# ryanelandt/PressureFieldContact.jl

Hardware: NVIDIA B200
Metric: contact_wrench_evals_per_sec (higher is better)
Workload: dtype f64

## Files before the change

pressurefieldcontact.jl_b200/csrc/pfc_clip.cuh:

```cuda
#pragma once
#include "pfc_math.cuh"
#include "pfc_types.cuh"

namespace pfc {

template <class T> struct Zeta { T c[4]; };

template <class T> PFC_D Zeta<T> clip_node(const Zeta<T>& z_non, const Zeta<T>& z_pos, int i) {
    const T w1 = z_non.c[i], w2 = z_pos.c[i];
    const T inv = 1.0 / (w1 - w2);
    const T c1 = w1 * inv, c2 = w2 * inv;
    Zeta<T> r;
#pragma unroll
    for (int k = 0; k < 4; ++k) r.c[k] = c1 * z_pos.c[k] - c2 * z_non.c[k];
    return r;
}

template <class T> __device__ __noinline__ int clip_tet(Zeta<T>* z, int n, int& flags) {
    for (int i = 0; i < 4; ++i) {
        bool all_non_pos = true, all_non_neg = true;
        unsigned non_pos = 0;
        for (int k = 0; k < n; ++k) {
            const double s = val(z[k].c[i]);
            const bool np = (s <= 0.0);
            non_pos |= (np ? 1u : 0u) << k;
            all_non_pos = all_non_pos && np;
            all_non_neg = all_non_neg && (0.0 <= s);
        }
        if (all_non_pos) return 0;
        if (all_non_neg) continue;
        int k0 = -1;
        for (int k = 0; k < n; ++k) {
            const int k1 = (k + 1 == n) ? 0 : k + 1;
            if (((non_pos >> k) & 1u) && !((non_pos >> k1) & 1u)) { k0 = k; break; }
        }
        if (k0 < 0) { flags |= kFlagNonFinite; return 0; }
        Zeta<T> w[8];
        for (int j = 0; j < n; ++j) { int k = k0 + j; if (k >= n) k -= n; w[j] = z[k]; }
        int m = n;
        while (m > 3 && val(w[m - 2].c[i]) <= 0.0) --m;
        const Zeta<T> z_start = clip_node(w[0], w[1], i);
        const double last = val(w[m - 1].c[i]);
        const bool last_inside = (m <= 5) ? (0.0 < last) : (0.0 <= last);
        z[0] = z_start;
        if (last_inside) {
            for (int k = 1; k < m; ++k) z[k] = w[k];
            z[m] = clip_node(w[0], w[m - 1], i);
            n = m + 1;
        } else {
            for (int k = 1; k < m - 1; ++k) z[k] = w[k];
            z[m - 1] = clip_node(w[m - 1], w[m - 2], i);
            n = m;
        }
        if (m == 7) return n;
    }
    return n;
}

PFC_D void clip_node_inplace(const double* zn, const double* zp, double w1, double w2, double* r) {
    const double inv = 1.0 / (w1 - w2);
    const double c1 = w1 * inv, c2 = w2 * inv;
#pragma unroll
    for (int k = 0; k < 4; ++k) r[k] = c1 * zp[k] - c2 * zn[k];
}
PFC_D int clip_tet_inplace(double* z, int n, int& flags) {
#pragma unroll 1
    for (int i = 0; i < 4; ++i) {
        unsigned np = 0, nn = 0, ps = 0;
        for (int k = 0; k < n; ++k) {
            const double s = z[4 * k + i];
            np |= (s <= 0.0 ? 1u : 0u) << k;
            nn |= (0.0 <= s ? 1u : 0u) << k;
            ps |= (0.0 < s ? 1u : 0u) << k;
        }
        const unsigned full = (1u << n) - 1u;
        if (np == full) return 0;
        if (nn == full) continue;
        const unsigned trans = np & ~(((np >> 1) | (np << (n - 1))) & full);
        if (!trans) { flags |= kFlagNonFinite; return 0; }
        const int k0 = __ffs(trans) - 1;
        const unsigned rnp = ((np >> k0) | (np << (n - k0))) & full;
        const unsigned rnn = ((nn >> k0) | (nn << (n - k0))) & full;
        const unsigned rps = ((ps >> k0) | (ps << (n - k0))) & full;
        int m = n;
        while (m > 3 && ((rnp >> (m - 2)) & 1u)) --m;
        const bool last_inside = (((m <= 5) ? rps : rnn) >> (m - 1)) & 1u;
        const int keep_end = last_inside ? m - 1 : m - 2;
        double w0[4], w1[4], wa[4], wb[4], zs[4], ze[4];
        {
            const int i1 = (k0 + 1 < n) ? k0 + 1 : k0 + 1 - n;
            const int ja = last_inside ? 0 : m - 1, jb = last_inside ? m - 1 : m - 2;
            const int ia = (k0 + ja < n) ? k0 + ja : k0 + ja - n, ib = (k0 + jb < n) ? k0 + jb : k0 + jb - n;
#pragma unroll
            for (int c = 0; c < 4; ++c) { w0[c] = z[4 * k0 + c]; w1[c] = z[4 * i1 + c]; wa[c] = z[4 * ia + c]; wb[c] = z[4 * ib + c]; }
            clip_node_inplace(w0, w1, z[4 * k0 + i], z[4 * i1 + i], zs);
            clip_node_inplace(wa, wb, z[4 * ia + i], z[4 * ib + i], ze);
        }
        if (k0 != 0) {
#pragma unroll 1
            for (int c = 0; c < 4; ++c) {
                double t[7];
#pragma unroll
                for (int j = 1; j <= 7; ++j)
                    if (j <= keep_end) { const int idx = (k0 + j < n) ? k0 + j : k0 + j - n; t[j - 1] = z[4 * idx + c]; }
#pragma unroll
                for (int j = 1; j <= 7; ++j)
                    if (j <= keep_end) z[4 * j + c] = t[j - 1];
            }
        }
#pragma unroll
        for (int c = 0; c < 4; ++c) { z[c] = zs[c]; z[4 * (keep_end + 1) + c] = ze[c]; }
        n = keep_end + 2;
        if (m == 7) return n;
    }
    return n;
}

template <class T> PFC_D void zero_small(Zeta<T>* z, int n) {
    for (int k = 0; k < n; ++k)
#pragma unroll
        for (int i = 0; i < 4; ++i) {
            const bool keep = 1.0e-14 < fabs(val(z[k].c[i]));
            z[k].c[i] = z[k].c[i] * (keep ? 1.0 : 0.0);
        }
}

template <class T> PFC_D Vec3<T> weight_poly(const Vec3<T>& p1, const Vec3<T>& p2, const T& w1, const T& w2) {
    const T inv = 1.0 / (w1 - w2);
    const T c1 = w1 * inv, c2 = w2 * inv;
    return mk<T>(c1 * p2.x - c2 * p1.x, c1 * p2.y - c2 * p1.y, c1 * p2.z - c2 * p1.z);
}

template <class T> __device__ __noinline__ int plane_tet(const T* plane, const Vec3<T>* v, Vec3<T>* out) {
    T proj[4];
    int n_neg = 0, n_pos = 0;
    unsigned pos = 0, neg = 0;
#pragma unroll
    for (int k = 0; k < 4; ++k) {
        proj[k] = plane[0] * v[k].x + plane[1] * v[k].y + plane[2] * v[k].z + plane[3];
        const double p = val(proj[k]);
        if (p < 0.0) { ++n_neg; neg |= 1u << k; }
        if (0.0 < p) { ++n_pos; pos |= 1u << k; }
    }
    if (n_pos == 0 || n_neg == 0) return 0;
    const signed char TRI[4][3][2] = {{{1, 0}, {3, 0}, {2, 0}}, {{0, 1}, {2, 1}, {3, 1}}, {{0, 2}, {3, 2}, {1, 2}}, {{0, 3}, {1, 3}, {2, 3}}};
    const signed char QUAD[3][4][2] = {{{1, 2}, {1, 3}, {0, 3}, {0, 2}}, {{0, 1}, {0, 3}, {2, 3}, {2, 1}}, {{0, 2}, {0, 1}, {3, 1}, {3, 2}}};
    int cnt, sel;
    bool forward;
    if (n_pos == 1) { sel = __ffs(pos) - 1; cnt = 3; forward = true; }
    else if (n_neg == 1) { sel = __ffs(neg) - 1; cnt = 3; forward = false; }
    else {
        const unsigned p0 = pos & 1u;
        if (((pos >> 1) & 1u) == p0) sel = 0;
        else if (((pos >> 2) & 1u) == p0) sel = 1;
        else if (((pos >> 3) & 1u) == p0) sel = 2;
        else return 0;
        cnt = 4;
        forward = (0.0 < val(proj[0]));
    }
    for (int k = 0; k < cnt; ++k) {
        const int i1 = (cnt == 3) ? TRI[sel][k][0] : QUAD[sel][k][0];
        const int i2 = (cnt == 3) ? TRI[sel][k][1] : QUAD[sel][k][1];
        const Vec3<T> p = weight_poly(v[i1], v[i2], proj[i1], proj[i2]);
        out[forward ? k : cnt - 1 - k] = p;
    }
    return cnt;
}

}
```

pressurefieldcontact.jl_b200/csrc/pfc_large.cu:

```cuda
#include <algorithm>
#include <cstddef>
#include <cstdio>
#include <cstdlib>
#include <vector>

#include <cuda_pipeline_primitives.h>

#include "pfc_exact.h"
#include "pfc_large.h"
#include "pfc_patch.cuh"
#include "pfc_sat.cuh"

namespace pfc {

namespace {

#define LCU(call)                         \
    do {                                  \
        cudaError_t e_ = (call);          \
        if (e_ != cudaSuccess) return e_; \
    } while (0)

constexpr int kStackCap = 1024;
constexpr int kDfsWarps = 4;
// ... 419 lines not shown
        unsigned incl = s;
#pragma unroll
        for (int o = 1; o < 32; o <<= 1) { const unsigned v = __shfl_up_sync(0xffffffffu, incl, o); if (lane >= o) incl += v; }
        unsigned run = incl - s;
#pragma unroll
        for (int j = 0; j < 8; ++j) { base[wib][8 * lane + j] = run + hist[(size_t)(8 * lane + j) * cap_tiles + tile]; run += t[j]; }
    }
    __syncwarp();
    const unsigned beg = tile * kTile, end = min(beg + kTile, n);
    constexpr int B = 8;
    for (unsigned c0 = beg; c0 < end; c0 += 32 * B) {
        unsigned long long kk[B]; unsigned vv[B];
#pragma unroll
        for (int j = 0; j < B; ++j) { const unsigned i = c0 + 32 * j + lane; const bool ok = i < end; kk[j] = ok ? keys_in[i] : 0ull; vv[j] = ok ? vals_in[i] : 0u; }
#pragma unroll
        for (int j = 0; j < B; ++j) {
            const unsigned i = c0 + 32 * j + lane;
            const bool valid = i < end;
            const unsigned d = valid ? (unsigned)((kk[j] >> shift) & 255u) : 256u + lane;
            const unsigned peers = __match_any_sync(0xffffffffu, d);
            const unsigned rank = __popc(peers & ((1u << lane) - 1u));
            unsigned pos = 0;
            if (valid) pos = base[wib][d] + rank;
            __syncwarp();
            if (valid && rank == (unsigned)__popc(peers) - 1) base[wib][d] = pos + 1;
            __syncwarp();
            if (valid) { keys_out[pos] = kk[j]; vals_out[pos] = vv[j]; }
        }
    }
}

__global__ void __launch_bounds__(1024) small_sort_kernel(const unsigned long long* keys_in, const unsigned* vals_in, Counters* cnt, unsigned cap_pairs,
                                                          unsigned long long* keys_out, unsigned* vals_out, int radix_queued) {
    extern __shared__ __align__(16) unsigned char sort_smem[];
    const unsigned n = listed_pairs(cnt, cap_pairs);
    if (n > kSmallSort && !radix_queued && threadIdx.x == 0) atomicOr(&cnt->overflow, 8u);
    if (n == 0 || n > kSmallSort) return;
    unsigned m = 1;
    while (m < n) m <<= 1;
    unsigned long long* k = reinterpret_cast<unsigned long long*>(sort_smem);
    unsigned* v = reinterpret_cast<unsigned*>(k + m);
    for (unsigned i = threadIdx.x; i < m; i += blockDim.x) { k[i] = i < n ? keys_in[i] : ~0ull; v[i] = i < n ? vals_in[i] : 0u; }
    __syncthreads();
    for (unsigned size = 2; size <= m; size <<= 1)
        for (unsigned stride = size >> 1; stride > 0; stride >>= 1) {
            for (unsigned t = threadIdx.x; t < m / 2; t += blockDim.x) {
                const unsigned lo = 2 * t - (t & (stride - 1)), hi = lo + stride;
                const bool up = (lo & size) == 0;
                const unsigned long long a = k[lo], b = k[hi];
                if ((a > b) == up) { k[lo] = b; k[hi] = a; const unsigned tv = v[lo]; v[lo] = v[hi]; v[hi] = tv; }
            }
            __syncthreads();
        }
    for (unsigned i = threadIdx.x; i < n; i += blockDim.x) { keys_out[i] = k[i]; vals_out[i] = v[i]; }
}

__global__ void gather_sorted_kernel(const int3* __restrict__ pairs, const unsigned* __restrict__ vals, const Counters* cnt, unsigned cap_pairs, int3* sorted,
                                     unsigned* seg_start, unsigned* seg_end) {
    const unsigned n = listed_pairs(cnt, cap_pairs);
    for (unsigned i = blockIdx.x * blockDim.x + threadIdx.x; i < n; i += gridDim.x * blockDim.x) {
        const int3 p = pairs[vals[i]];
        sorted[i] = p;
        const int prev = i > 0 ? pairs[vals[i - 1]].x : -1;
        if (p.x != prev) { seg_start[p.x] = i; if (prev >= 0) seg_end[prev] = i; }
        if (i == n - 1) seg_end[p.x] = n;
    }
}
__global__ void __launch_bounds__(1024) units_scan_kernel(const unsigned* __restrict__ seg_start, const unsigned* __restrict__ seg_end, unsigned n_prob, unsigned* unit_start,
                                                          Counters* cnt, unsigned shard_rank, unsigned shard_world) {
    __shared__ unsigned warp_sums[32];
    __shared__ unsigned carry;
    if (threadIdx.x == 0) carry = 0;
    __syncthreads();
    const int lane = threadIdx.x & 31, w = threadIdx.x >> 5;
    for (unsigned base = 0; base < n_prob; base += 1024) {
        const unsigned i = base + threadIdx.x;
        const unsigned v = i < n_prob ? (seg_end[i] - seg_start[i] + kChunk - 1) / kChunk : 0;
        unsigned incl = v;
#pragma unroll
        for (int o = 1; o < 32; o <<= 1) { const unsigned t = __shfl_up_sync(0xffffffffu, incl, o); if (lane >= o) incl += t; }
        if (lane == 31) warp_sums[w] = incl;
        __syncthreads();
        if (w == 0) {
            unsigned s = warp_sums[lane];
#pragma unroll
            for (int o = 1; o < 32; o <<= 1) { const unsigned t = __shfl_up_sync(0xffffffffu, s, o); if (lane >= o) s += t; }
            warp_sums[lane] = s;
        }
        __syncthreads();
        const unsigned before = carry + (w > 0 ? warp_sums[w - 1] : 0) + incl - v;
        if (i < n_prob) unit_start[i] = before;
        __syncthreads();
        if (threadIdx.x == 1023) carry = before + v;
        __syncthreads();
    }
    if (threadIdx.x == 0) { unit_start[n_prob] = carry; cnt->n_units = carry; }
    (void)shard_rank; (void)shard_world;
}

constexpr int kLPolyStride = 35;
static_assert(sizeof(PolyRec<double>) == kLPolyStride * sizeof(double), "PolyRec<double> is 35 doubles");
struct NarrowLargeSmem {
    double poly[kChunk * kLPolyStride];
    double item_res[kChunk * 7];
    PatchCtx<double> cx;
    double fpv[8];
    double tot[8];
    unsigned short items[kChunk * 8];
    int2 slot_pair[kChunk];
    unsigned char slot_n[kChunk];
    int warp_tot[kChunk / 32];
    int s_prob;
    int pflags;
};

__global__ void __launch_bounds__(kChunk, 2) narrow_large_kernel(SceneDev sc, LargeScene ls, EvalIO io, const int3* __restrict__ sorted, const unsigned* __restrict__ seg_start,
                                                                 const unsigned* __restrict__ seg_end, const unsigned* __restrict__ unit_start, unsigned n_prob,
                                                                 const Counters* cnt, double* chunk_out, int* chunk_points, int* prob_flags) {
    extern __shared__ __align__(16) unsigned char smem_raw[];
    NarrowLargeSmem& sm = *reinterpret_cast<NarrowLargeSmem*>(smem_raw);
    const unsigned n_units = cnt->n_units;
    const int tid = threadIdx.x, lane = tid & 31, wib = tid >> 5;
    constexpr int NW = kChunk / 32;
    for (unsigned u = blockIdx.x; u < n_units; u += gridDim.x) {
        if (tid == 0) {
            unsigned lo = 0, hi = n_prob;
            while (hi - lo > 1) { const unsigned mid = (lo + hi) >> 1; if (unit_start[mid] <= u) lo = mid; else hi = mid; }
            sm.s_prob = (int)lo;
            sm.pflags = 0;
        }
        __syncthreads();
        const int p = sm.s_prob;
        long long env; int k;
        prob_to_ei(sc, ls, p, env, k);
        const InsDev& ins = sc.ins[k];
        if (ins.model != PFC_MODEL_REGULARIZED) { __syncthreads(); continue; }
        const long long ei = env * sc.n_ins + k;
        if (wib == 0) {
            const double* X = io.X + 16 * ei;
            const double* twist = io.twist + 6 * ei;
            PatchCtx<double>& cx = sm.cx;
            if (lane < 8) sm.fpv[lane] = ins.p[lane];
            if (lane < 9) { const int i = lane / 3, j = lane % 3; cx.x21.r[lane] = X[4 * j + i]; }
            else if (lane < 12) cx.x21.t[lane - 9] = X[12 + lane - 9];
            else if (lane < 21) { const int e = lane - 12, i = e / 3, j = e % 3; cx.x12.r[e] = X[4 * i + j]; }
            else if (lane < 24) { const int i = lane - 21; cx.x12.t[i] = -(X[4 * i] * X[12] + X[4 * i + 1] * X[13] + X[4 * i + 2] * X[14]); }
            else if (lane < 27) (&cx.w_ang.x)[lane - 24] = twist[lane - 24];
            else if (lane < 30) (&cx.w_lin.x)[lane - 27] = twist[lane - 24];
            else if (lane == 30) { cx.chi = ins.chi; cx.Ebar1 = ins.Ebar1; cx.Ebar2 = ins.Ebar2; cx.n_quad = ins.n_quad; }
            if (lane < 8) sm.tot[lane] = 0.0;
        }
        __syncthreads();
        const unsigned i = seg_start[p] + (u - unit_start[p]) * kChunk + tid;
        double zr[16];
        int n0 = 0;
        int3 pr = make_int3(0, 0, 0);
        if (i < seg_end[p]) {
            pr = sorted[i];
            n0 = start_polygon_zeta(sc, ins, pr.y, pr.z, sm.cx, zr);
        }
        const unsigned alive = __ballot_sync(0xffffffffu, n0 > 0);
        if (lane == 0) sm.warp_tot[wib] = __popc(alive);
        __syncthreads();
        int before = 0, n_slot = 0;
#pragma unroll
        for (int w = 0; w < NW; ++w) { const int t = sm.warp_tot[w]; if (w < wib) before += t; n_slot += t; }
        if (n0 > 0) {
            const int slot = before + __popc(alive & ((1u << lane) - 1u));
            double* z = sm.poly + slot * kLPolyStride;
#pragma unroll
            for (int j = 0; j < 16; ++j)
                if (j < 4 * n0) z[j] = zr[j];
            sm.slot_pair[slot] = make_int2(pr.y, pr.z); sm.slot_n[slot] = (unsigned char)n0;
        }
        __syncthreads();
        int nv = 0;
        if (tid < n_slot) {
            const int2 e = sm.slot_pair[tid];
            PolyRec<double>& out = *reinterpret_cast<PolyRec<double>*>(sm.poly + tid * kLPolyStride);
            int flags = 0;
            const int n = clip_tet_inplace(reinterpret_cast<double*>(&out), (int)sm.slot_n[tid], flags);
            if (n >= 3) {
                finish_polygon_slot(n, sc.tets[ins.prim_base2 + e.y], pair_normal(sc, ins, e.x, e.y, sm.cx), out);
                nv = n;
            }
            if (flags) atomicOr(&sm.pflags, flags);
        }
        int incl = nv;
#pragma unroll
        for (int o = 1; o < 32; o <<= 1) { const int v = __shfl_up_sync(0xffffffffu, incl, o); if (lane >= o) incl += v; }
        __syncthreads();
        if (lane == 31) sm.warp_tot[wib] = incl;
        __syncthreads();
        int ibefore = 0, total = 0;
#pragma unroll
        for (int w = 0; w < NW; ++w) { const int t = sm.warp_tot[w]; if (w < wib) ibefore += t; total += t; }
        const int at = ibefore + incl - nv;
        for (int q = 0; q < nv; ++q) sm.items[at + q] = (unsigned short)((tid << 3) | q);
        __syncthreads();
        for (int i0 = 0; i0 < total; i0 += kChunk) {
            const int i1 = min(total, i0 + kChunk);
            const int it = i0 + tid;
            if (it < i1) {
                const int code = sm.items[it];
                const int slot = code >> 3, q = code & 7;
                const PolyRec<double>& prc = *reinterpret_cast<const PolyRec<double>*>(sm.poly + slot * kLPolyStride);
                Accum<double, 6> tmp;
                tmp.fp = sm.fpv; tmp.w_ang = sm.cx.w_ang; tmp.w_lin = sm.cx.w_lin; tmp.dump = nullptr; tmp.dump_cap = 0;
                tmp.reset(ACC_REGULARIZED);
                const int qp = (q == 0) ? prc.n - 1 : q - 1;
                integrate_subtri(prc.v[qp], prc.v[q], prc.cen, prc.nrm, prc.eps_r, sm.cx, tmp);
                double* res = sm.item_res + tid * 7;
#pragma unroll
                for (int j = 0; j < 6; ++j) res[j] = tmp.a[j];
                reinterpret_cast<int*>(res + 6)[0] = tmp.n_points;
            }
            __syncthreads();
            if (wib == 0) {
                double part[6] = {0.0, 0.0, 0.0, 0.0, 0.0, 0.0};
                int part_n = 0;
                for (int j = lane; j < i1 - i0; j += 32) {
                    const double* res = sm.item_res + j * 7;
#pragma unroll
                    for (int c = 0; c < 6; ++c) part[c] += res[c];
                    part_n += reinterpret_cast<const int*>(res + 6)[0];
                }
                int pn = part_n;
#pragma unroll
                for (int o = 16; o > 0; o >>= 1) pn += __shfl_xor_sync(0xffffffffu, pn, o);
                double mine = (double)pn;
#pragma unroll
                for (int c = 0; c < 6; ++c) { const double t = warp_sum(part[c]); mine = (lane == c) ? t : mine; }
                if (lane < 7) sm.tot[lane] += mine;
            }
            __syncthreads();
        }
        if (tid < kNA) chunk_out[(size_t)u * kNA + tid] = sm.tot[tid];
        if (tid == 0) { chunk_points[u] = (int)sm.tot[6]; if (sm.pflags) atomicOr(&prob_flags[p], sm.pflags); }
        __syncthreads();
    }
}

__global__ void __launch_bounds__(128) finish_large_kernel(SceneDev sc, LargeScene ls, EvalIO io, const unsigned* __restrict__ seg_start, const unsigned* __restrict__ seg_end,
                                                           const unsigned* __restrict__ unit_start, unsigned n_prob, const double* __restrict__ chunk_out,
                                                           const int* __restrict__ chunk_points, const int* __restrict__ prob_flags, double* part_out, int apply_parts) {
    const int lane = threadIdx.x & 31, wib = threadIdx.x >> 5;
    for (unsigned p = blockIdx.x * 4 + wib; p < n_prob; p += gridDim.x * 4) {
        long long env; int k;
        prob_to_ei(sc, ls, (int)p, env, k);
        const InsDev& ins = sc.ins[k];
        const long long ei = env * sc.n_ins + k;
        if (ins.model == PFC_MODEL_BRISTLE) {
            if (lane == 0 && !apply_parts) { io.n_pairs[ei] = (long long)seg_end[p] - (long long)seg_start[p]; io.flags[ei] = prob_flags[p]; }
            if (lane == 0 && part_out && !apply_parts) for (int j = 0; j < kLargePartStride; ++j) part_out[(size_t)p * kLargePartStride + j] = 0.0;
            continue;
        }
        double sum[kNA];
        int pts = 0;
        if (apply_parts) {
            for (int j = 0; j < kNA; ++j) sum[j] = part_out[(size_t)p * kLargePartStride + j];
            pts = (int)part_out[(size_t)p * kLargePartStride + kNA];
        } else {
            const unsigned c0 = unit_start[p], c1 = unit_start[p + 1];
            for (int j = 0; j < kNA; ++j) sum[j] = 0.0;
            for (unsigned c = c0 + lane; c < c1; c += 32) {
                for (int j = 0; j < kNA; ++j) sum[j] += chunk_out[(size_t)c * kNA + j];
                pts += chunk_points[c];
            }
            for (int j = 0; j < kNA; ++j) sum[j] = warp_sum(sum[j]);
#pragma unroll
            for (int o = 16; o > 0; o >>= 1) pts += __shfl_xor_sync(0xffffffffu, pts, o);
            if (part_out) {
                if (lane == 0) {
                    for (int j = 0; j < kNA; ++j) part_out[(size_t)p * kLargePartStride + j] = sum[j];
                    part_out[(size_t)p * kLargePartStride + kNA] = (double)pts;
                    part_out[(size_t)p * kLargePartStride + kNA + 1] = (double)(seg_end[p] - seg_start[p]);
                }
                continue;
            }
        }
        const long long n_pairs = apply_parts ? (long long)part_out[(size_t)p * kLargePartStride + kNA + 1] : (long long)seg_end[p] - (long long)seg_start[p];
        if (lane == 0) {
            const bool contact = pts > 0;
            double* wo = io.wrench + 6 * ei;
            for (int j = 0; j < 6; ++j) wo[j] = contact ? sum[j] : 0.0;
            io.n_pairs[ei] = n_pairs;
            io.flags[ei] = prob_flags[p] | (contact ? kFlagContact : 0);
        }
    }
}

__global__ void zero_int_kernel(int* p, unsigned n) {
    for (unsigned i = blockIdx.x * blockDim.x + threadIdx.x; i < n; i += gridDim.x * blockDim.x) p[i] = 0;
}
__global__ void init_segments_kernel(unsigned* seg_start, unsigned* seg_end, unsigned n) {
    for (unsigned i = blockIdx.x * blockDim.x + threadIdx.x; i < n; i += gridDim.x * blockDim.x) { seg_start[i] = 0; seg_end[i] = 0; }
}

template <class T> cudaError_t ensure(T*& p, size_t& cap, size_t need) {
    if (need <= cap) return cudaSuccess;
    alloc_generation()++;
    if (p) cudaFree(p);
    p = nullptr; cap = 0;
    cudaError_t e = cudaMalloc(&p, need * sizeof(T));
    if (e != cudaSuccess) return e;
    cap = need;
    return cudaMemset(p, 0, need * sizeof(T));
// ... 240 lines not shown
```

pressurefieldcontact.jl_b200/csrc/pfc_patch.cuh:

```cuda
#pragma once
#include "pfc_clip.cuh"
#include "pfc_math.cuh"
#include "pfc_types.cuh"

namespace pfc {

#define PFC_Q1 0.33333333333333331483
#define PFC_QA 0.16666666666666674068
#define PFC_QB 0.66666666666666651864

enum AccMode { ACC_REGULARIZED = 0, ACC_DUMP = 4 };

template <class T> struct PatchCtx {
    Xform<T> x21;
    Xform<T> x12;
    Vec3<T> w_ang, w_lin;
    double chi, Ebar1, Ebar2;
    int n_quad;
};

template <class T> struct PolyRec {
    Vec3<T> v[8];
    Vec3<T> nrm;
    Vec3<T> cen;
// ... 81 lines not shown
    quad_point(v1, v2, cen, nrm, g0, g1, g2, g3, PFC_QA, PFC_QA, PFC_QB, dA, cx, acc);
}

template <class T> PFC_D void finish_polygon(const Zeta<T>* z, int n, const TetRec& tet, PolyRec<T>& out) {
    out.n = n;
    for (int k = 0; k < n; ++k) {
        const T z0 = z[k].c[0], z1 = z[k].c[1], z2 = z[k].c[2], z3 = z[k].c[3];
        out.v[k] = mk<T>(tet.v[0] * z0 + tet.v[3] * z1 + tet.v[6] * z2 + tet.v[9] * z3, tet.v[1] * z0 + tet.v[4] * z1 + tet.v[7] * z2 + tet.v[10] * z3,
                         tet.v[2] * z0 + tet.v[5] * z1 + tet.v[8] * z2 + tet.v[11] * z3);
    }
    T cum_sum = T(0.0);
    Vec3<T> cum = mk<T>(T(0.0), T(0.0), T(0.0));
    for (int k = 2; k < n; ++k) {
        const Vec3<T> a = out.v[0], b = out.v[k - 1], c = out.v[k];
        const T area = dot(out.nrm, cross(b - a, c - b) * 0.5);
        cum = cum + ((a + b + c) * (1.0 / 3.0)) * area;
        cum_sum += area;
    }
    out.cen = out.v[0];
    if (val(cum_sum) != 0.0) { const T inv = 1.0 / cum_sum; out.cen = mk<T>(cum.x * inv, cum.y * inv, cum.z * inv); }
#pragma unroll
    for (int k = 0; k < 4; ++k) out.eps_r[k] = tet.eps_r[k];
}

template <class T> PFC_D bool clip_tri_tet(const TriRec& tri, const TetRec& tet, const PatchCtx<T>& cx, PolyRec<T>& out, int& flags) {
    Zeta<T> z[8];
#pragma unroll
    for (int k = 0; k < 3; ++k) {
        const Vec3<T> p = apply_d(cx.x21, mk<double>(tri.v[3 * k], tri.v[3 * k + 1], tri.v[3 * k + 2]));
#pragma unroll
        for (int i = 0; i < 4; ++i) z[k].c[i] = tet.inv[4 * i] * p.x + tet.inv[4 * i + 1] * p.y + tet.inv[4 * i + 2] * p.z + tet.inv[4 * i + 3];
    }
    const int n = clip_tet(z, 3, flags);
    if (n < 3) return false;
    out.nrm = rot_d(cx.x21, mk<double>(tri.n[0], tri.n[1], tri.n[2]));
    finish_polygon(z, n, tet, out);
    return true;
}

template <class T> PFC_D bool clip_tet_tet(const TetRec& t1, const TetRec& t2, const PatchCtx<T>& cx, PolyRec<T>& out, int& flags) {
    T plane[4];
    {
        const double g0 = cx.Ebar1 * t1.eps_r[0], g1 = cx.Ebar1 * t1.eps_r[1], g2 = cx.Ebar1 * t1.eps_r[2], g3 = cx.Ebar1 * t1.eps_r[3];
        const Xform<T>& Y = cx.x12;
        const T p0 = g0 * Y.r[0] + g1 * Y.r[3] + g2 * Y.r[6];
        const T p1 = g0 * Y.r[1] + g1 * Y.r[4] + g2 * Y.r[7];
        const T p2 = g0 * Y.r[2] + g1 * Y.r[5] + g2 * Y.r[8];
        const T p3 = g0 * Y.t[0] + g1 * Y.t[1] + g2 * Y.t[2] + g3;
        plane[0] = cx.Ebar2 * t2.eps_r[0] - p0;
        plane[1] = cx.Ebar2 * t2.eps_r[1] - p1;
        plane[2] = cx.Ebar2 * t2.eps_r[2] - p2;
        plane[3] = cx.Ebar2 * t2.eps_r[3] - p3;
    }
    Vec3<T> v[4], poly[4];
#pragma unroll
    for (int k = 0; k < 4; ++k) v[k] = apply_d(cx.x21, mk<double>(t1.v[3 * k], t1.v[3 * k + 1], t1.v[3 * k + 2]));
    const int n0 = plane_tet(plane, v, poly);
    if (n0 < 3) return false;
    Zeta<T> z[8];
    for (int k = 0; k < n0; ++k)
#pragma unroll
        for (int i = 0; i < 4; ++i)
            z[k].c[i] = t2.inv[4 * i] * poly[k].x + t2.inv[4 * i + 1] * poly[k].y + t2.inv[4 * i + 2] * poly[k].z + t2.inv[4 * i + 3];
    zero_small(z, n0);
    const int n = clip_tet(z, n0, flags);
    if (n < 3) return false;
    const T inv_len = 1.0 / sqrt_(plane[0] * plane[0] + plane[1] * plane[1] + plane[2] * plane[2]);
    out.nrm = mk<T>(plane[0] * inv_len, plane[1] * inv_len, plane[2] * inv_len);
    finish_polygon(z, n, t2, out);
    return true;
}

template <class T> PFC_D bool prefilter_pair(const SceneDev& sc, const InsDev& ins, int prim1, int prim2, const PatchCtx<T>& cx) {
    const TetRec& t2 = sc.tets[ins.prim_base2 + prim2];
    if (ins.kind1 == 0) {
        const TriRec& tri = sc.tris[ins.prim_base1 + prim1];
        unsigned all_non_pos = 0xfu;
#pragma unroll
        for (int k = 0; k < 3; ++k) {
            const Vec3<T> p = apply_d(cx.x21, mk<double>(tri.v[3 * k], tri.v[3 * k + 1], tri.v[3 * k + 2]));
#pragma unroll
            for (int i = 0; i < 4; ++i) {
                const T z = t2.inv[4 * i] * p.x + t2.inv[4 * i + 1] * p.y + t2.inv[4 * i + 2] * p.z + t2.inv[4 * i + 3];
                if (!(val(z) <= 0.0)) all_non_pos &= ~(1u << i);
            }
        }
        return all_non_pos == 0;
    }
    const TetRec& t1 = sc.tets[ins.prim_base1 + prim1];
    const double g0 = cx.Ebar1 * t1.eps_r[0], g1 = cx.Ebar1 * t1.eps_r[1], g2 = cx.Ebar1 * t1.eps_r[2], g3 = cx.Ebar1 * t1.eps_r[3];
    const Xform<T>& Y = cx.x12;
    const T pl0 = cx.Ebar2 * t2.eps_r[0] - (g0 * Y.r[0] + g1 * Y.r[3] + g2 * Y.r[6]);
    const T pl1 = cx.Ebar2 * t2.eps_r[1] - (g0 * Y.r[1] + g1 * Y.r[4] + g2 * Y.r[7]);
    const T pl2 = cx.Ebar2 * t2.eps_r[2] - (g0 * Y.r[2] + g1 * Y.r[5] + g2 * Y.r[8]);
    const T pl3 = cx.Ebar2 * t2.eps_r[3] - (g0 * Y.t[0] + g1 * Y.t[1] + g2 * Y.t[2] + g3);
    int n_pos = 0, n_neg = 0;
#pragma unroll
    for (int k = 0; k < 4; ++k) {
        const Vec3<T> v = apply_d(cx.x21, mk<double>(t1.v[3 * k], t1.v[3 * k + 1], t1.v[3 * k + 2]));
        const double pr = val(pl0 * v.x + pl1 * v.y + pl2 * v.z + pl3);
        n_pos += (0.0 < pr); n_neg += (pr < 0.0);
    }
    return n_pos != 0 && n_neg != 0;
}

template <class T> PFC_D bool clip_pair(const SceneDev& sc, const InsDev& ins, int prim1, int prim2, const PatchCtx<T>& cx, PolyRec<T>& out, int& flags) {
    const TetRec& t2 = sc.tets[ins.prim_base2 + prim2];
    if (ins.kind1 == 0) return clip_tri_tet(sc.tris[ins.prim_base1 + prim1], t2, cx, out, flags);
    return clip_tet_tet(sc.tets[ins.prim_base1 + prim1], t2, cx, out, flags);
}

PFC_D bool finish_polygon_slot(int n, const TetRec& tet_g, const Vec3<double>& nrm, PolyRec<double>& out) {
    double* z = reinterpret_cast<double*>(&out);
    struct { double v[12]; } tet;
    load_wide<12>(tet_g.v, tet.v);
    for (int k = 0; k < n; ++k) {
        const double z0 = z[4 * k], z1 = z[4 * k + 1], z2 = z[4 * k + 2], z3 = z[4 * k + 3];
        out.v[k] = mk<double>(tet.v[0] * z0 + tet.v[3] * z1 + tet.v[6] * z2 + tet.v[9] * z3, tet.v[1] * z0 + tet.v[4] * z1 + tet.v[7] * z2 + tet.v[10] * z3,
                              tet.v[2] * z0 + tet.v[5] * z1 + tet.v[8] * z2 + tet.v[11] * z3);
    }
    double cum_sum = 0.0;
    Vec3<double> cum = mk<double>(0.0, 0.0, 0.0);
    const Vec3<double> a = out.v[0];
    Vec3<double> b = out.v[1];
    for (int k = 2; k < n; ++k) {
        const Vec3<double> c = out.v[k];
        const double area = dot(nrm, cross(b - a, c - b) * 0.5);
        cum = cum + ((a + b + c) * (1.0 / 3.0)) * area;
        cum_sum += area;
        b = c;
    }
    Vec3<double> cen = a;
    if (cum_sum != 0.0) { const double inv = 1.0 / cum_sum; cen = mk<double>(cum.x * inv, cum.y * inv, cum.z * inv); }
    out.nrm = nrm;
    out.cen = cen;
    load_wide<4>(tet_g.eps_r, out.eps_r);
    out.n = n;
    return true;
}

PFC_D int start_polygon_zeta(const SceneDev& sc, const InsDev& ins, int prim1, int prim2, const PatchCtx<double>& cx, double* zr) {
    const TetRec& t2 = sc.tets[ins.prim_base2 + prim2];
    if (ins.kind1 == 0) {
        struct { double v[9]; double n[3]; } tri;
        struct { double inv[16]; } t2r;
        load_wide<12>(sc.tris[ins.prim_base1 + prim1].v, tri.v);
        load_wide<16>(t2.inv, t2r.inv);
        unsigned all_non_pos = 0xfu;
#pragma unroll
        for (int k = 0; k < 3; ++k) {
            const Vec3<double> p = apply_d(cx.x21, mk<double>(tri.v[3 * k], tri.v[3 * k + 1], tri.v[3 * k + 2]));
#pragma unroll
            for (int i = 0; i < 4; ++i) {
                zr[4 * k + i] = t2r.inv[4 * i] * p.x + t2r.inv[4 * i + 1] * p.y + t2r.inv[4 * i + 2] * p.z + t2r.inv[4 * i + 3];
                if (!(zr[4 * k + i] <= 0.0)) all_non_pos &= ~(1u << i);
            }
        }
        return all_non_pos ? 0 : 3;
    }
    const TetRec& t1 = sc.tets[ins.prim_base1 + prim1];
    double plane[4];
    {
        const double g0 = cx.Ebar1 * t1.eps_r[0], g1 = cx.Ebar1 * t1.eps_r[1], g2 = cx.Ebar1 * t1.eps_r[2], g3 = cx.Ebar1 * t1.eps_r[3];
        const Xform<double>& Y = cx.x12;
        plane[0] = cx.Ebar2 * t2.eps_r[0] - (g0 * Y.r[0] + g1 * Y.r[3] + g2 * Y.r[6]);
        plane[1] = cx.Ebar2 * t2.eps_r[1] - (g0 * Y.r[1] + g1 * Y.r[4] + g2 * Y.r[7]);
        plane[2] = cx.Ebar2 * t2.eps_r[2] - (g0 * Y.r[2] + g1 * Y.r[5] + g2 * Y.r[8]);
        plane[3] = cx.Ebar2 * t2.eps_r[3] - (g0 * Y.t[0] + g1 * Y.t[1] + g2 * Y.t[2] + g3);
    }
    Vec3<double> v[4], poly[4];
#pragma unroll
    for (int k = 0; k < 4; ++k) v[k] = apply_d(cx.x21, mk<double>(t1.v[3 * k], t1.v[3 * k + 1], t1.v[3 * k + 2]));
    const int n0 = plane_tet(plane, v, poly);
    if (n0 < 3) return 0;
#pragma unroll
    for (int k = 0; k < 4; ++k)
        if (k < n0) {
#pragma unroll
            for (int i = 0; i < 4; ++i) {
                const double zz = t2.inv[4 * i] * poly[k].x + t2.inv[4 * i + 1] * poly[k].y + t2.inv[4 * i + 2] * poly[k].z + t2.inv[4 * i + 3];
                zr[4 * k + i] = zz * ((1.0e-14 < fabs(zz)) ? 1.0 : 0.0);
            }
        }
    return n0;
}

PFC_D Vec3<double> pair_normal(const SceneDev& sc, const InsDev& ins, int prim1, int prim2, const PatchCtx<double>& cx) {
    if (ins.kind1 == 0) {
        const TriRec& tri = sc.tris[ins.prim_base1 + prim1];
        return rot_d(cx.x21, mk<double>(tri.n[0], tri.n[1], tri.n[2]));
    }
    const TetRec& t1 = sc.tets[ins.prim_base1 + prim1];
    const TetRec& t2 = sc.tets[ins.prim_base2 + prim2];
    const double g0 = cx.Ebar1 * t1.eps_r[0], g1 = cx.Ebar1 * t1.eps_r[1], g2 = cx.Ebar1 * t1.eps_r[2];
    const Xform<double>& Y = cx.x12;
    const double p0 = cx.Ebar2 * t2.eps_r[0] - (g0 * Y.r[0] + g1 * Y.r[3] + g2 * Y.r[6]);
    const double p1 = cx.Ebar2 * t2.eps_r[1] - (g0 * Y.r[1] + g1 * Y.r[4] + g2 * Y.r[7]);
    const double p2 = cx.Ebar2 * t2.eps_r[2] - (g0 * Y.r[2] + g1 * Y.r[5] + g2 * Y.r[8]);
    const double inv_len = 1.0 / sqrt(p0 * p0 + p1 * p1 + p2 * p2);
    return mk<double>(p0 * inv_len, p1 * inv_len, p2 * inv_len);
}

template <class T, int NA> PFC_D void integrate_pair(const SceneDev& sc, const InsDev& ins, int prim1, int prim2, const PatchCtx<T>& cx, Accum<T, NA>& acc, int& flags) {
    PolyRec<T> pr;
    if (!clip_pair(sc, ins, prim1, prim2, cx, pr, flags)) return;
    Vec3<T> v2 = pr.v[pr.n - 1];
    for (int k = 0; k < pr.n; ++k) {
        const Vec3<T> v1 = v2;
        v2 = pr.v[k];
        integrate_subtri(v1, v2, pr.cen, pr.nrm, pr.eps_r, cx, acc);
    }
}

}
```

pressurefieldcontact.jl_b200/csrc/pfc_small.cu:

```cuda
#include <cstdlib>

#include "pfc_launch.h"
#include "pfc_patch.cuh"
#include "pfc_sat.cuh"

namespace pfc {

namespace {

constexpr unsigned kDone = 0x80000000u;
PFC_D unsigned enc(int a, int b) { return (unsigned(a) << 15) | unsigned(b); }
PFC_D int dec_a(unsigned e) { return int((e >> 15) & 0x7fffu); }
PFC_D int dec_b(unsigned e) { return int(e & 0x7fffu); }

PFC_D int warp_sum_int(int x) {
#pragma unroll
    for (int o = 16; o > 0; o >>= 1) x += __shfl_xor_sync(0xffffffffu, x, o);
    return x;
}
PFC_D int warp_incl_scan(int x, int lane) {
#pragma unroll
    for (int o = 1; o < 32; o <<= 1) { const int v = __shfl_up_sync(0xffffffffu, x, o); if (lane >= o) x += v; }
    return x;
}
// ... 78 lines not shown
#pragma unroll
        for (int q = 0; q < P; ++q) dead |= (q >= n_valid ? 1u : 0u) << q;
        int pc[P + 1];
        for (;;) {
            const int* pcs = pre + cur * (P + 1);
            int* pn = pre + (cur ^ 1) * (P + 1);
            const unsigned* fc = front + (size_t)cur * fcap;
            unsigned* fn = front + (size_t)(cur ^ 1) * fcap;
            const unsigned short* olc = olist + (size_t)cur * fcap;
            unsigned short* oln = olist + (size_t)(cur ^ 1) * fcap;
            pc[0] = 0;
#pragma unroll
            for (int q = 0; q < P; ++q) {
                pc[q + 1] = ((dead >> q) & 1u) ? pc[q] : pcs[q + 1];
                if (pc[q + 1] == pc[q]) dead |= 1u << q;
            }
            const int total = pc[P];
            if (n_open == 0) break;
            for (int j = lane; j < n_open; j += T) {
                const int c = olc[j];
                int q = 0;
#pragma unroll
                for (int r = 1; r < P; ++r) q += (c >= pc[r]);
                const unsigned e = fc[c];
                const int ia = dec_a(e), ib = dec_b(e);
                const InsDev& ins = sc.ins[s_ins[q]];
                const NodeRec& a = *reinterpret_cast<const NodeRec*>(ntab + (size_t)nstride * (ins.node_base1 + ia));
                const NodeRec& b = *reinterpret_cast<const NodeRec*>(ntab + (size_t)nstride * (ins.node_base2 + ib));
                SatA A;
                sat_prepare_a<false>(a, xf + 12 * q, xf + 12 * q + 9, A);
                int code = 0;
                if (sat_test<false>(A, b)) code = (a.kind < 0) ? ((b.kind < 0) ? 1 : 2) : ((b.kind < 0) ? 3 : 4);
                res[c] = (unsigned char)code;
            }
            __syncwarp();
            int carry = 0;
            for (int c0 = 0; c0 < total; c0 += T) {
                const int c = c0 + lane;
                int cnt = 0, ocnt = 0, q = 0;
                unsigned ch0 = 0, ch1 = 0, ch2 = 0, ch3 = 0;
                if (c < total) {
#pragma unroll
                    for (int r = 1; r < P; ++r) q += (c >= pc[r]);
                    const unsigned e = fc[c];
                    if (e & kDone) { cnt = 1; ch0 = e; }
                    else {
                        const int code = res[c];
                        if (code) {
                            const int ia = dec_a(e), ib = dec_b(e);
                            const InsDev& ins = sc.ins[s_ins[q]];
                            const NodeRec& a = *reinterpret_cast<const NodeRec*>(ntab + (size_t)nstride * (ins.node_base1 + ia));
                            const NodeRec& b = *reinterpret_cast<const NodeRec*>(ntab + (size_t)nstride * (ins.node_base2 + ib));
                            const int al = ia + 1, ar = a.right, bl = ib + 1, br = b.right;
                            if (code == 1) { cnt = 1; ch0 = kDone | enc(ar, br); }
                            else if (code == 2) { cnt = ocnt = 2; ch0 = enc(ia, bl); ch1 = enc(ia, br); }
                            else if (code == 3) { cnt = ocnt = 2; ch0 = enc(al, ib); ch1 = enc(ar, ib); }
                            else { cnt = ocnt = 4; ch0 = enc(al, bl); ch1 = enc(ar, bl); ch2 = enc(al, br); ch3 = enc(ar, br); }
                        }
                    }
                }
                const int mine = cnt | (ocnt << 16);
                int incl = mine;
#pragma unroll
                for (int o = 1; o < 32; o <<= 1) { const int v = __shfl_up_sync(0xffffffffu, incl, o); if (lane >= o) incl += v; }
                const int chunk_total = __shfl_sync(0xffffffffu, incl, 31);
                const int excl = carry + incl - mine;
                const int at = excl & 0xffff, oat = excl >> 16;
                if (at + cnt <= fcap) {
                    if (cnt > 0) fn[at] = ch0;
                    if (cnt > 1) fn[at + 1] = ch1;
                    if (cnt > 2) { fn[at + 2] = ch2; fn[at + 3] = ch3; }
                    for (int k = 0; k < ocnt; ++k) oln[oat + k] = (unsigned short)(at + k);
                }
                tile_overflow |= __any_sync(0xffffffffu, cnt > 0 && at + cnt > fcap);
                if (c < total) {
                    int end_q = pc[P];
#pragma unroll
                    for (int r = 1; r < P; ++r) if (r == q + 1) end_q = pc[r];
                    if (c + 1 == end_q) pn[q + 1] = min(at + cnt, fcap);
                }
                carry += chunk_total;
            }
            n_open = carry >> 16;
            __syncwarp();
            cur ^= 1;
            if (tile_overflow) break;
        }
        if (tile_overflow) {
#pragma unroll
            for (int q = 0; q < P; ++q)
                if (lane == q && s_ei[q] >= 0) {
                    io.n_pairs[s_ei[q]] = 0;
                    io.flags[s_ei[q]] = kFlagOverflow;
                    if (sc.ins_overflow) sc.ins_overflow[s_ins[q]] = 1;
                }
            __syncwarp();
            continue;
        }
        {
            const unsigned* fc = front + (size_t)cur * fcap;
            const int total = pc[P];
            for (int c = lane; c < total; c += T) {
                int q = 0;
#pragma unroll
                for (int r = 1; r < P; ++r) q += (c >= pc[r]);
                int beg_q = 0;
#pragma unroll
                for (int r = 1; r < P; ++r) if (r == q) beg_q = pc[r];
                const int i = c - beg_q;
                const unsigned e = fc[c];
                if (i < cap) pairs_out[(size_t)cap * s_ei[q] + i] = e;
                if (io.dbg_pairs && i < io.dbg_cap) {
                    int* out = io.dbg_pairs + 2 * ((long long)io.dbg_cap * s_ei[q] + i);
                    out[0] = dec_a(e); out[1] = dec_b(e);
                }
            }
#pragma unroll
            for (int o = 16; o > 0; o >>= 1) flags |= __shfl_xor_sync(0xffffffffu, flags, o);
#pragma unroll
            for (int q = 0; q < P; ++q)
                if (lane == q && s_ei[q] >= 0) {
                    const int n = pc[q + 1] - pc[q];
                    io.n_pairs[s_ei[q]] = n < cap ? n : cap;
                    if (n > cap && sc.ins_overflow) { sc.ins_overflow[s_ins[q]] = 1; flags |= kFlagOverflow; }
                    io.flags[s_ei[q]] = flags;
                }
        }
        __syncwarp();
    }
}

constexpr int kPolyStride = 35;
static_assert(sizeof(PolyRec<double>) == kPolyStride * sizeof(double), "PolyRec<double> is 35 doubles");

template <int P> struct TileSmem {
    static constexpr int kThreads = 32 * P;
    double poly[kThreads * kPolyStride];
    PatchCtx<double> cx[P];
    long long ei[P];
    const double* fp[P];
    int ins[P];
    int n_cand[P];
    double wtot[P][P][8];
    int warp_tot[P];
    int pflags[P];
    unsigned short items[kThreads * 8];
    unsigned char poly_prob[kThreads];
    unsigned slot_pair[kThreads];
    unsigned char slot_n[kThreads];
    int resume_c;
    long long next_tile;
    double fpv[P][8];
};
static_assert(sizeof(TileSmem<4>) <= 45 * 1024, "5 CTAs per SM need <= 45 KB each");

template <int P, int MINB>
__global__ void __launch_bounds__(32 * P, MINB) narrow_tile_kernel(SceneDev sc, EvalIO io, int cap, const unsigned* __restrict__ pairs_in, unsigned* __restrict__ ticket) {
    constexpr int kTileThreads = 32 * P;
    extern __shared__ __align__(16) unsigned char smem_raw[];
    TileSmem<P>& sm = *reinterpret_cast<TileSmem<P>*>(smem_raw);
    const int tid = threadIdx.x, lane = tid & 31, wib = tid >> 5;
    const long long n_prob = io.n_env * sc.n_small;
    const long long n_tile = (n_prob + P - 1) / P;
    const int sum_q = wib;
    for (long long tile = blockIdx.x; tile < n_tile;) {
        {
            const long long prob = tile * P + wib;
            const long long env = prob < n_prob ? prob / sc.n_small : 0;
            const int k = prob < n_prob ? sc.small_ins[prob - env * sc.n_small] : 0;
            if (prob < n_prob && sc.ins[k].model == PFC_MODEL_REGULARIZED) {
                const InsDev& ins = sc.ins[k];
                const long long ei = env * sc.n_ins + k;
                const double* X = io.X + 16 * ei;
                const double* twist = io.twist + 6 * ei;
                PatchCtx<double>& cx = sm.cx[wib];
                if (lane < 8) sm.fpv[wib][lane] = ins.p[lane];
                if (lane < 9) { const int i = lane / 3, j = lane % 3; cx.x21.r[lane] = X[4 * j + i]; }
                else if (lane < 12) cx.x21.t[lane - 9] = X[12 + lane - 9];
                else if (lane < 21) { const int e = lane - 12, i = e / 3, j = e % 3; cx.x12.r[e] = X[4 * i + j]; }
                else if (lane < 24) { const int i = lane - 21; cx.x12.t[i] = -(X[4 * i] * X[12] + X[4 * i + 1] * X[13] + X[4 * i + 2] * X[14]); }
                else if (lane < 27) (&cx.w_ang.x)[lane - 24] = twist[lane - 24];
                else if (lane < 30) (&cx.w_lin.x)[lane - 27] = twist[lane - 24];
                else if (lane == 30) { cx.chi = ins.chi; cx.Ebar1 = ins.Ebar1; cx.Ebar2 = ins.Ebar2; cx.n_quad = ins.n_quad; }
                else { sm.ei[wib] = ei; sm.fp[wib] = sm.fpv[wib]; sm.ins[wib] = k; sm.n_cand[wib] = (int)io.n_pairs[ei]; sm.pflags[wib] = 0; }
            } else if (lane == 31) { sm.ei[wib] = -1; sm.n_cand[wib] = 0; sm.ins[wib] = 0; sm.fp[wib] = nullptr; sm.pflags[wib] = 0; }
        }
        __syncthreads();
        if (tid == 0) sm.next_tile = (long long)gridDim.x + atomicAdd(ticket, 1u);
        int pre[P + 1];
        pre[0] = 0;
#pragma unroll
        for (int q = 0; q < P; ++q) pre[q + 1] = pre[q] + sm.n_cand[q];
        const int n_cand = pre[P];
        for (int j = lane; j < P * 8; j += 32) sm.wtot[wib][j >> 3][j & 7] = 0.0;
        int filled = 0;
        int c0 = 0;
        while (true) {
            if (c0 < n_cand) {
                const int c = c0 + tid;
                double zr[16];
                int n0 = 0, q = 0;
                unsigned e = 0;
                if (c < n_cand) {
                    int first = 0;
#pragma unroll
                    for (int r = 1; r < P; ++r) { const bool ge = c >= pre[r]; q += ge; first = ge ? pre[r] : first; }
                    e = pairs_in[(size_t)cap * sm.ei[q] + (c - first)];
                    n0 = start_polygon_zeta(sc, sc.ins[sm.ins[q]], dec_a(e), dec_b(e), sm.cx[q], zr);
                }
                const unsigned alive = __ballot_sync(0xffffffffu, n0 > 0);
                if (lane == 0) sm.warp_tot[wib] = __popc(alive);
                __syncthreads();
                int before = 0, round_total = 0;
#pragma unroll
                for (int w = 0; w < P; ++w) { const int t = sm.warp_tot[w]; if (w < wib) before += t; round_total += t; }
                if (n0 > 0) {
                    const int slot = filled + before + __popc(alive & ((1u << lane) - 1u));
                    if (slot < kTileThreads) {
                        double* z = sm.poly + slot * kPolyStride;
#pragma unroll
                        for (int j = 0; j < 16; ++j)
                            if (j < 4 * n0) z[j] = zr[j];
                        sm.slot_pair[slot] = e; sm.slot_n[slot] = (unsigned char)n0; sm.poly_prob[slot] = (unsigned char)q;
                    } else if (slot == kTileThreads) sm.resume_c = c;
                }
                __syncthreads();
                if (filled + round_total > kTileThreads) { filled = kTileThreads; c0 = sm.resume_c; }
                else { filled += round_total; c0 += kTileThreads; }
            }
            const bool last = c0 >= n_cand;
            if (filled == 0) { if (last) break; continue; }
            if (filled < kTileThreads && !last) continue;
            const int batch_n = filled;
            int nv = 0;
            if (tid < batch_n) {
                const int q = sm.poly_prob[tid];
                const unsigned e = sm.slot_pair[tid];
                PolyRec<double>& out = *reinterpret_cast<PolyRec<double>*>(sm.poly + tid * kPolyStride);
                int flags = 0;
                const int n = clip_tet_inplace(reinterpret_cast<double*>(&out), (int)sm.slot_n[tid], flags);
                if (n >= 3) {
                    const InsDev& ins = sc.ins[sm.ins[q]];
                    finish_polygon_slot(n, sc.tets[ins.prim_base2 + dec_b(e)], pair_normal(sc, ins, dec_a(e), dec_b(e), sm.cx[q]), out);
                    nv = n;
                }
                if (flags) atomicOr(&sm.pflags[q], flags);
            }
            int incl = nv;
#pragma unroll
            for (int o = 1; o < 32; o <<= 1) { const int v = __shfl_up_sync(0xffffffffu, incl, o); if (lane >= o) incl += v; }
            if (lane == 31) sm.warp_tot[wib] = incl;
            __syncthreads();
            int before = 0, total = 0;
#pragma unroll
            for (int w = 0; w < P; ++w) { const int t = sm.warp_tot[w]; if (w < wib) before += t; total += t; }
            const int at = before + incl - nv;
            for (int k = 0; k < nv; ++k) sm.items[at + k] = (unsigned short)((tid << 3) | k);
            __syncthreads();
            for (int i0 = 0; i0 < total; i0 += kTileThreads) {
                const int it = i0 + tid;
                double a6[6] = {0.0, 0.0, 0.0, 0.0, 0.0, 0.0};
                int npts = 0, q = -1;
                if (it < total) {
                    const int code = sm.items[it];
                    const int slot = code >> 3, k = code & 7;
                    const PolyRec<double>& pr = *reinterpret_cast<const PolyRec<double>*>(sm.poly + slot * kPolyStride);
                    q = sm.poly_prob[slot];
                    const PatchCtx<double>& cx = sm.cx[q];
                    Accum<double, 6> tmp;
                    tmp.fp = sm.fpv[q]; tmp.w_ang = cx.w_ang; tmp.w_lin = cx.w_lin; tmp.dump = nullptr; tmp.dump_cap = 0;
                    tmp.reset(ACC_REGULARIZED);
                    const int kp = (k == 0) ? pr.n - 1 : k - 1;
                    integrate_subtri(pr.v[kp], pr.v[k], pr.cen, pr.nrm, pr.eps_r, cx, tmp);
#pragma unroll
                    for (int j = 0; j < 6; ++j) a6[j] = tmp.a[j];
                    npts = tmp.n_points;
                }
                const unsigned act = __ballot_sync(0xffffffffu, it < total);
                if (act) {
                    const int q_first = __shfl_sync(0xffffffffu, q, __ffs(act) - 1), q_last = __shfl_sync(0xffffffffu, q, 31 - __clz(act));
                    for (int qq = q_first; qq <= q_last; ++qq) {
                        const bool mine_q = q == qq;
                        double mine = (double)warp_sum_int(mine_q ? npts : 0);
#pragma unroll
                        for (int j = 0; j < 6; ++j) { const double t = warp_sum(mine_q ? a6[j] : 0.0); mine = (lane == j) ? t : mine; }
                        if (lane < 7) sm.wtot[wib][qq][lane] += mine;
                    }
                }
            }
            __syncthreads();
            filled = 0;
            if (last) break;
        }
        __syncthreads();
        {
            const long long ei = sm.ei[sum_q];
            if (ei >= 0) {
                double t = 0.0;
                if (lane < 7) {
#pragma unroll
                    for (int w = 0; w < P; ++w) t += sm.wtot[w][sum_q][lane];
                }
                const bool contact = __shfl_sync(0xffffffffu, t, 6) > 0.0;
                if (lane < 6) io.wrench[6 * ei + lane] = contact ? t : 0.0;
                if (lane == 6) io.flags[ei] |= sm.pflags[sum_q] | (contact ? kFlagContact : 0);
            }
        }
        __syncthreads();
        tile = sm.next_tile;
    }
}

__global__ void dump_traction_kernel(SceneDev sc, EvalIO io, long long env, int k, const int* pairs, long long n_pairs, double* out, int cap, int* n_points) {
    const InsDev& ins = sc.ins[k];
    const long long ei = env * sc.n_ins + k;
    PatchCtx<double> cx;
    load_xform(io.X + 16 * ei, cx.x21);
    cx.x12 = inverse(cx.x21);
    const double* tw = io.twist + 6 * ei;
    cx.w_ang = mk<double>(tw[0], tw[1], tw[2]);
    cx.w_lin = mk<double>(tw[3], tw[4], tw[5]);
    cx.chi = ins.chi; cx.Ebar1 = ins.Ebar1; cx.Ebar2 = ins.Ebar2; cx.n_quad = ins.n_quad;
    Accum<double> acc;
    acc.fp = ins.p; acc.w_ang = cx.w_ang; acc.w_lin = cx.w_lin; acc.dump = out; acc.dump_cap = cap;
    acc.reset(ACC_DUMP);
    int flags = 0;
    for (long long i = 0; i < n_pairs; ++i) integrate_pair(sc, ins, pairs[2 * i], pairs[2 * i + 1], cx, acc, flags);
    *n_points = acc.n_points;
}

}

int persistent_blocks(const void* kern, int threads, size_t smem, cudaError_t* err) {
    int per_sm = 0, dev = 0, n_sm = 0;
    *err = cudaFuncSetAttribute(kern, cudaFuncAttributeMaxDynamicSharedMemorySize, (int)smem);
    if (*err != cudaSuccess) return 0;
    cudaGetDevice(&dev);
    cudaDeviceGetAttribute(&n_sm, cudaDevAttrMultiProcessorCount, dev);
    *err = cudaOccupancyMaxActiveBlocksPerMultiprocessor(&per_sm, kern, threads, smem);
    return n_sm * (per_sm > 0 ? per_sm : 1);
}

namespace {

template <int P, int NW, int MINB>
cudaError_t launch_broad_tile(const SceneDev& sc, const EvalIO& io, int cap, unsigned* pairs, cudaStream_t stream) {
    struct Tag {};
    auto kern = broad_tile_kernel<P, NW, MINB>;
    const int n_stage = sc.small_node_n <= kNodeTabMax ? sc.small_node_n : 0;
    const size_t smem = BroadTileLayout<P>::bytes(cap, NW, n_stage);
    int cached_blocks;
    {
        std::lock_guard<std::mutex> g(launch_mutex());
        LaunchSlot& sl = launch_slot<Tag>();
        if (sl.key0 != cap || sl.key1 != n_stage) {
            cudaError_t e;
            sl.blocks = persistent_blocks((const void*)kern, 32 * NW, smem, &e);
            if (e != cudaSuccess) return e;
            sl.key0 = cap; sl.key1 = n_stage;
// ... 85 lines not shown
```

Measured before the change: 18.91 million.

## Cut register pressure: inline plane-tet clipping, stage polygons in shared memory

Replaces the noinline plane_tet call with an inlined version that takes lambdas. Vertices are computed on demand and emitted directly into zeta coordinates, and the edge tables become packed constexpr bitmasks, so the local Vec3 arrays go away. The per-thread zr[16] buffer now points into the shared-memory poly slot instead of a register or local array. The prefix-sum array is dropped and recomputed from shared memory, and lane and wib are re-derived behind an asm barrier to shorten their live ranges. The shared-memory budget assert is relaxed to 56 KB (4 CTAs/SM), which may lower occupancy and adds shared-memory traffic for zr.

```diff
diff --git a/pressurefieldcontact.jl_b200/csrc/pfc_clip.cuh b/pressurefieldcontact.jl_b200/csrc/pfc_clip.cuh
--- a/pressurefieldcontact.jl_b200/csrc/pfc_clip.cuh
+++ b/pressurefieldcontact.jl_b200/csrc/pfc_clip.cuh
@@ -131,20 +131,33 @@
     return mk<T>(c1 * p2.x - c2 * p1.x, c1 * p2.y - c2 * p1.y, c1 * p2.z - c2 * p1.z);
 }
 
-template <class T> __device__ __noinline__ int plane_tet(const T* plane, const Vec3<T>* v, Vec3<T>* out) {
+constexpr signed char kPlaneTetTri[4][3][2] = {{{1, 0}, {3, 0}, {2, 0}}, {{0, 1}, {2, 1}, {3, 1}}, {{0, 2}, {3, 2}, {1, 2}}, {{0, 3}, {1, 3}, {2, 3}}};
+constexpr signed char kPlaneTetQuad[3][4][2] = {{{1, 2}, {1, 3}, {0, 3}, {0, 2}}, {{0, 1}, {0, 3}, {2, 3}, {2, 1}}, {{0, 2}, {0, 1}, {3, 1}, {3, 2}}};
+constexpr unsigned long long plane_tet_edge_bits(bool quad) {
+    unsigned long long b = 0;
+    for (int s = 0; s < (quad ? 3 : 4); ++s)
+        for (int k = 0; k < (quad ? 4 : 3); ++k) {
+            const signed char* e = quad ? kPlaneTetQuad[s][k] : kPlaneTetTri[s][k];
+            b |= (unsigned long long)(e[0] | e[1] << 2) << (4 * ((quad ? 4 : 3) * s + k));
+        }
+    return b;
+}
+constexpr unsigned long long kPlaneTetTriBits = plane_tet_edge_bits(false), kPlaneTetQuadBits = plane_tet_edge_bits(true);
+template <class T> PFC_D T pick4(int i, const T& a, const T& b, const T& c, const T& d) { return i == 0 ? a : i == 1 ? b : i == 2 ? c : d; }
+
+template <class T, class Vert, class Emit> PFC_D int plane_tet_inline(const T* plane, Vert&& vert, Emit&& emit) {
     T proj[4];
     int n_neg = 0, n_pos = 0;
     unsigned pos = 0, neg = 0;
 #pragma unroll
     for (int k = 0; k < 4; ++k) {
-        proj[k] = plane[0] * v[k].x + plane[1] * v[k].y + plane[2] * v[k].z + plane[3];
+        const Vec3<T> v = vert(k);
+        proj[k] = plane[0] * v.x + plane[1] * v.y + plane[2] * v.z + plane[3];
         const double p = val(proj[k]);
         if (p < 0.0) { ++n_neg; neg |= 1u << k; }
         if (0.0 < p) { ++n_pos; pos |= 1u << k; }
     }
     if (n_pos == 0 || n_neg == 0) return 0;
-    const signed char TRI[4][3][2] = {{{1, 0}, {3, 0}, {2, 0}}, {{0, 1}, {2, 1}, {3, 1}}, {{0, 2}, {3, 2}, {1, 2}}, {{0, 3}, {1, 3}, {2, 3}}};
-    const signed char QUAD[3][4][2] = {{{1, 2}, {1, 3}, {0, 3}, {0, 2}}, {{0, 1}, {0, 3}, {2, 3}, {2, 1}}, {{0, 2}, {0, 1}, {3, 1}, {3, 2}}};
     int cnt, sel;
     bool forward;
     if (n_pos == 1) { sel = __ffs(pos) - 1; cnt = 3; forward = true; }
@@ -158,13 +171,19 @@
         cnt = 4;
         forward = (0.0 < val(proj[0]));
     }
-    for (int k = 0; k < cnt; ++k) {
-        const int i1 = (cnt == 3) ? TRI[sel][k][0] : QUAD[sel][k][0];
-        const int i2 = (cnt == 3) ? TRI[sel][k][1] : QUAD[sel][k][1];
-        const Vec3<T> p = weight_poly(v[i1], v[i2], proj[i1], proj[i2]);
-        out[forward ? k : cnt - 1 - k] = p;
-    }
+    const unsigned long long edges = (cnt == 3) ? kPlaneTetTriBits : kPlaneTetQuadBits;
+#pragma unroll
+    for (int j = 0; j < 4; ++j)
+        if (j < cnt) {
+            const int k = forward ? j : cnt - 1 - j;
+            const unsigned e = unsigned(edges >> (4 * (cnt * sel + k))) & 15u;
+            const int i1 = e & 3u, i2 = e >> 2;
+            emit(j, weight_poly(vert(i1), vert(i2), pick4(i1, proj[0], proj[1], proj[2], proj[3]), pick4(i2, proj[0], proj[1], proj[2], proj[3])));
+        }
     return cnt;
+}
+template <class T> __device__ __noinline__ int plane_tet(const T* plane, const Vec3<T>* v, Vec3<T>* out) {
+    return plane_tet_inline(plane, [&](int k) { return v[k]; }, [&](int j, const Vec3<T>& p) { out[j] = p; });
 }
 
 }
diff --git a/pressurefieldcontact.jl_b200/csrc/pfc_large.cu b/pressurefieldcontact.jl_b200/csrc/pfc_large.cu
--- a/pressurefieldcontact.jl_b200/csrc/pfc_large.cu
+++ b/pressurefieldcontact.jl_b200/csrc/pfc_large.cu
@@ -595,7 +595,7 @@
         }
         __syncthreads();
         const unsigned i = seg_start[p] + (u - unit_start[p]) * kChunk + tid;
-        double zr[16];
+        double* zr = sm.poly + tid * kLPolyStride + 16;
         int n0 = 0;
         int3 pr = make_int3(0, 0, 0);
         if (i < seg_end[p]) {
diff --git a/pressurefieldcontact.jl_b200/csrc/pfc_patch.cuh b/pressurefieldcontact.jl_b200/csrc/pfc_patch.cuh
--- a/pressurefieldcontact.jl_b200/csrc/pfc_patch.cuh
+++ b/pressurefieldcontact.jl_b200/csrc/pfc_patch.cuh
@@ -257,8 +257,9 @@
             const Vec3<double> p = apply_d(cx.x21, mk<double>(tri.v[3 * k], tri.v[3 * k + 1], tri.v[3 * k + 2]));
 #pragma unroll
             for (int i = 0; i < 4; ++i) {
-                zr[4 * k + i] = t2r.inv[4 * i] * p.x + t2r.inv[4 * i + 1] * p.y + t2r.inv[4 * i + 2] * p.z + t2r.inv[4 * i + 3];
-                if (!(zr[4 * k + i] <= 0.0)) all_non_pos &= ~(1u << i);
+                const double zz = t2r.inv[4 * i] * p.x + t2r.inv[4 * i + 1] * p.y + t2r.inv[4 * i + 2] * p.z + t2r.inv[4 * i + 3];
+                zr[4 * k + i] = zz;
+                if (!(zz <= 0.0)) all_non_pos &= ~(1u << i);
             }
         }
         return all_non_pos ? 0 : 3;
@@ -273,21 +274,15 @@
         plane[2] = cx.Ebar2 * t2.eps_r[2] - (g0 * Y.r[2] + g1 * Y.r[5] + g2 * Y.r[8]);
         plane[3] = cx.Ebar2 * t2.eps_r[3] - (g0 * Y.t[0] + g1 * Y.t[1] + g2 * Y.t[2] + g3);
     }
-    Vec3<double> v[4], poly[4];
-#pragma unroll
-    for (int k = 0; k < 4; ++k) v[k] = apply_d(cx.x21, mk<double>(t1.v[3 * k], t1.v[3 * k + 1], t1.v[3 * k + 2]));
-    const int n0 = plane_tet(plane, v, poly);
-    if (n0 < 3) return 0;
-#pragma unroll
-    for (int k = 0; k < 4; ++k)
-        if (k < n0) {
-#pragma unroll
-            for (int i = 0; i < 4; ++i) {
-                const double zz = t2.inv[4 * i] * poly[k].x + t2.inv[4 * i + 1] * poly[k].y + t2.inv[4 * i + 2] * poly[k].z + t2.inv[4 * i + 3];
-                zr[4 * k + i] = zz * ((1.0e-14 < fabs(zz)) ? 1.0 : 0.0);
-            }
+    const auto vert = [&](int k) { return apply_d(cx.x21, mk<double>(t1.v[3 * k], t1.v[3 * k + 1], t1.v[3 * k + 2])); };
+    const int n0 = plane_tet_inline(plane, vert, [&](int k, const Vec3<double>& p) {
+#pragma unroll
+        for (int i = 0; i < 4; ++i) {
+            const double zz = t2.inv[4 * i] * p.x + t2.inv[4 * i + 1] * p.y + t2.inv[4 * i + 2] * p.z + t2.inv[4 * i + 3];
+            zr[4 * k + i] = zz * ((1.0e-14 < fabs(zz)) ? 1.0 : 0.0);
         }
-    return n0;
+    });
+    return n0 < 3 ? 0 : n0;
 }
 
 PFC_D Vec3<double> pair_normal(const SceneDev& sc, const InsDev& ins, int prim1, int prim2, const PatchCtx<double>& cx) {
diff --git a/pressurefieldcontact.jl_b200/csrc/pfc_small.cu b/pressurefieldcontact.jl_b200/csrc/pfc_small.cu
--- a/pressurefieldcontact.jl_b200/csrc/pfc_small.cu
+++ b/pressurefieldcontact.jl_b200/csrc/pfc_small.cu
@@ -254,7 +254,7 @@
     long long next_tile;
     double fpv[P][8];
 };
-static_assert(sizeof(TileSmem<4>) <= 45 * 1024, "5 CTAs per SM need <= 45 KB each");
+static_assert(sizeof(TileSmem<4>) <= 56 * 1024, "4 CTAs per SM need <= 56 KB each");
 
 template <int P, int MINB>
 __global__ void __launch_bounds__(32 * P, MINB) narrow_tile_kernel(SceneDev sc, EvalIO io, int cap, const unsigned* __restrict__ pairs_in, unsigned* __restrict__ ticket) {
@@ -267,6 +267,8 @@
     const int sum_q = wib;
     for (long long tile = blockIdx.x; tile < n_tile;) {
         {
+            int lane = tid & 31, wib = tid >> 5;
+            asm volatile("" : "+r"(lane), "+r"(wib));
             const long long prob = tile * P + wib;
             const long long env = prob < n_prob ? prob / sc.n_small : 0;
             const int k = prob < n_prob ? sc.small_ins[prob - env * sc.n_small] : 0;
@@ -289,24 +291,22 @@
         }
         __syncthreads();
         if (tid == 0) sm.next_tile = (long long)gridDim.x + atomicAdd(ticket, 1u);
-        int pre[P + 1];
-        pre[0] = 0;
-#pragma unroll
-        for (int q = 0; q < P; ++q) pre[q + 1] = pre[q] + sm.n_cand[q];
-        const int n_cand = pre[P];
+        int n_cand = 0;
+#pragma unroll
+        for (int q = 0; q < P; ++q) n_cand += sm.n_cand[q];
         for (int j = lane; j < P * 8; j += 32) sm.wtot[wib][j >> 3][j & 7] = 0.0;
         int filled = 0;
         int c0 = 0;
         while (true) {
             if (c0 < n_cand) {
                 const int c = c0 + tid;
-                double zr[16];
+                double* zr = sm.poly + tid * kPolyStride + 16;
                 int n0 = 0, q = 0;
                 unsigned e = 0;
                 if (c < n_cand) {
-                    int first = 0;
-#pragma unroll
-                    for (int r = 1; r < P; ++r) { const bool ge = c >= pre[r]; q += ge; first = ge ? pre[r] : first; }
+                    int first = 0, end = 0;
+#pragma unroll
+                    for (int r = 1; r < P; ++r) { end += sm.n_cand[r - 1]; const bool ge = c >= end; q += ge; first = ge ? end : first; }
                     e = pairs_in[(size_t)cap * sm.ei[q] + (c - first)];
                     n0 = start_polygon_zeta(sc, sc.ins[sm.ins[q]], dec_a(e), dec_b(e), sm.cx[q], zr);
                 }
```

New measurement: 19.95 million (median of 6 runs). +5.5%, better.
